# stanFurrer/Robust-Multimodal-Contrastive-Learning

Hardware: AMD Instinct MI355X
Metric: image-text pairs/sec, ViLT-B/32 RMCL step (PGD K=3) (higher is better)
Workload: dtype bf16; 1 GPU; RMCL step, PGD K=3 image attack + MoCo InfoNCE (queue 65536) + full backward + AdamW, ViLT-B/32, bs=64/GPU, 384x384 img + 40 tok (BASELINE configs[2]; [3] when n_gpus=8); global_batch=64, parallelism=dp1, grad_sync=ring/f32, ln_fold=on (shift-robust form)

## Files before the change

include/rmcl.h:

```cpp
#ifndef RMCL_H
#define RMCL_H
#include <stdint.h>
#ifdef __cplusplus
extern "C" {
#endif

#define RMCL_F32 0
#define RMCL_BF16 1

#define RMCL_MODE_INFER 0
#define RMCL_MODE_DATA 1
#define RMCL_MODE_FULL 2
#define RMCL_MODE_CLS_TAIL 16
#define RMCL_MODE_STREAM_ATTN 32

typedef struct rmcl_dims {
  int B;
  int L;
  int P;
  int D;
  int H;
  int layers;
  int mlp;
  int patch_k;
// ... 35 lines not shown
int rmcl_linear_lnfold_c(const void* xb, const void* wf, const float* s, const float* c, const float* part, int nparts, const float* center,
                         void* out, void* preact, int M, int N, int K, int gelu, float eps, float* mean, float* rstd, void* stream);

typedef struct rmcl_chain_stage {
  const void* A; const void* W; const float* bias; const float* residual; void* out; void* out2; float* part; const float* center;
  const float* ln_s; const float* ln_c; float* mean; float* rstd;
  int N, K, epi, nparts; float ln_eps;
} rmcl_chain_stage;
int rmcl_gemm_chain(const rmcl_chain_stage* stages, int n, int M, uint32_t* tickets, uint32_t epoch, int flags, int32_t* xcc, int64_t* stamps,
                    int stamp_wg, void* stream);

int rmcl_l2_prefetch_experiment(const void* A, int64_t lda_bytes, int M, int rows_per_tile, int tiles_per_xcd, int col_tiles, const void* W,
                                int64_t ldw_bytes, int nB, int nk, int tick, int lead, int per_xcd, int wgs, int* counter, int64_t* stamps,
                                void* stream);

typedef struct rmcl_layout {
  int64_t word, pos, btype, eln_w, eln_b;
  int64_t vtype;
  int64_t cls, pos_img, patch_w, patch_b;
  int64_t layer0, layer_stride;
  int64_t ln1_w, ln1_b, qkv_w, qkv_b, proj_w, proj_b, ln2_w, ln2_b, fc1_w, fc1_b, fc2_w, fc2_b;
  int64_t norm_w, norm_b;
  int64_t mh0_w, mh0_b, mh1_w, mh1_b, mh3_w;
  int64_t ema_end;
  int64_t pool_w, pool_b;
  int64_t itm_w, itm_b;
  int64_t total;
} rmcl_layout;

const char* rmcl_last_error(void);
int rmcl_version(void);

int rmcl_tune_set(int key, int value);

int rmcl_grad_ready_wait(int layer, void* stream);
int rmcl_set_side_stream(void* stream);
int rmcl_set_prefetch_stream(void* stream);

int rmcl_dropout_mask_apply(float* x, int64_t n, uint32_t drop_seed, int layer, int site, float drop_p, void* stream);

int rmcl_prof_begin(int tag_mask, int max_launches);
int rmcl_prof_end(double* ms_total, int64_t* launches, double* flops_total);

void rmcl_param_layout(const rmcl_dims* d, rmcl_layout* out);
int64_t rmcl_stash_bytes(const rmcl_dims* d, int mode);
int64_t rmcl_workspace_bytes(const rmcl_dims* d);
int64_t rmcl_heads_stash_bytes(const rmcl_dims* d);


int rmcl_im2patch_f32(const float* img, float* patches, int B, int C, int Hh, int Ww, int ps, int to_image, void* stream);

int rmcl_patch_select(const float* img, int B, int C, int Hh, int Ww, int ps, int32_t* sel, int32_t* counts, int32_t* hw, void* stream);
int rmcl_im2patch_sel(float* img, float* patches, const int32_t* sel, const int32_t* counts, int sel_ld, int B, int n, int C, int Hh,
                      int Ww, int ps, int to_image, void* stream);
int rmcl_image_u8_to_patches(const uint8_t* img, const int32_t* sizes, const int32_t* sel, const int32_t* counts, int sel_ld, int B, int n,
                             int Hmax, int Wmax, int patch_size, const float* lut, float* patches, void* stream);

int rmcl_image_resize_u8(const uint8_t* src, const int32_t* src_sizes, int B, int Hs, int Ws, const int32_t* dst_sizes, int Hd, int Wd,
                         const int32_t* hbounds, const int32_t* hk, int ksh, const int32_t* vbounds, const int32_t* vk, int ksv, uint8_t* tmp,
                         uint8_t* dst, void* stream);

#define RMCL_RA_AUTOCONTRAST 0
#define RMCL_RA_EQUALIZE 1
#define RMCL_RA_ROTATE 2
#define RMCL_RA_POSTERIZE 3
#define RMCL_RA_SOLARIZE 4
// ... 252 lines not shown
```

robust-multimodal-contrastive-learning_amd/_lib.py:

```python
import ctypes as C
import os

import torch

_HERE = os.path.dirname(os.path.abspath(__file__))
LIB_PATH = os.environ.get("RMCL_LIB") or os.path.join(_HERE, "lib", "librmcl_hip.so")

F32, BF16 = 0, 1
MODE_INFER, MODE_DATA, MODE_FULL = 0, 1, 2
MODE_CLS_TAIL = 16
MODE_STREAM_ATTN = 32
PGD_DELTA_ZERO, PGD_SUM_PREV = 1, 2
HEADS_NO_WGRAD = 1
OPTIM_ADAM, OPTIM_SGD = 1, 2
EPI_BIAS, EPI_GELU, EPI_SAVE_PREACT, EPI_RESIDUAL, EPI_DGELU, EPI_ATOMIC, EPI_ACCUM, EPI_TANH = 1, 2, 4, 8, 16, 32, 64, 128
EPI_LNFOLD, EPI_ROWSTAT = 2048, 4096


class Dims(C.Structure):
    _fields_ = [(n, C.c_int) for n in
                ("B", "L", "P", "D", "H", "layers", "mlp", "patch_k", "proj", "vocab", "dtype", "exact", "Pp", "n_types", "img_type")]


class Ragged(C.Structure):
# ... 65 lines not shown


class MetricOps(C.Structure):
    _fields_ = [("n_ops", C.c_int32), ("reserved", C.c_int32), ("op", MetricOp * METRIC_MAX_OPS)]


class RmclError(RuntimeError):
    pass


def _load():
    if not os.path.exists(LIB_PATH):
        raise RmclError(
            f"{LIB_PATH} is missing: build it with `python -c 'import __graft_entry__ as g; g.build()'` "
            "(hipcc --offload-arch=gfx950).  rmcl_amd has no CPU fallback.")
    lib = C.CDLL(LIB_PATH)
    lib.rmcl_last_error.restype = C.c_char_p
    for name in ("rmcl_stash_bytes", "rmcl_workspace_bytes", "rmcl_heads_stash_bytes", "rmcl_infonce_ws_bytes",
                 "rmcl_attention_scratch_elems", "rmcl_attention_stream_stat_elems", "rmcl_ln_fold_elems", "rmcl_bt_stash_floats", "rmcl_bt_loss_ws_floats",
                 "rmcl_vqa_stash_floats", "rmcl_mlm_ws_floats", "rmcl_mpp_ws_floats", "rmcl_randaug_scratch_bytes", "rmcl_grad_stats_ws_bytes"):
        getattr(lib, name).restype = C.c_int64
    lib.rmcl_grad_stats_ws_bytes.argtypes = [C.c_int64]
    lib.rmcl_randaug_scratch_bytes.argtypes = [C.c_int, C.c_int]
    lib.rmcl_randaug_u8.argtypes = [C.c_void_p, C.c_void_p, C.c_int, C.c_int, C.c_int, C.c_void_p, C.c_void_p, C.c_int, C.c_void_p, C.c_void_p, C.c_void_p, C.c_void_p]
    lib.rmcl_mpp_labels_u8.argtypes = [C.c_void_p, C.c_void_p, C.c_int, C.c_int, C.c_int, C.c_void_p, C.c_void_p, C.c_void_p, C.c_int, C.c_int, C.c_int,
                                       C.c_void_p, C.c_void_p]
    lib.rmcl_metrics_update.argtypes = [C.c_void_p, C.c_int, C.POINTER(MetricOps), C.c_void_p]
    return lib


lib = _load()

EXPORTS = (
    "rmcl_last_error", "rmcl_version", "rmcl_prof_begin", "rmcl_prof_end", "rmcl_tune_set", "rmcl_grad_ready_wait", "rmcl_set_side_stream", "rmcl_set_prefetch_stream", "rmcl_dropout_mask_apply", "rmcl_param_layout", "rmcl_ln_fold_elems", "rmcl_ln_fold", "rmcl_linear_rowstat", "rmcl_linear_lnfold", "rmcl_linear_rowstat_c", "rmcl_linear_lnfold_c", "rmcl_weight_transpose_bf16", "rmcl_stash_bytes", "rmcl_workspace_bytes",
    "rmcl_heads_stash_bytes", "rmcl_im2patch_f32", "rmcl_patch_select", "rmcl_im2patch_sel", "rmcl_image_u8_to_patches", "rmcl_image_resize_u8", "rmcl_randaug_scratch_bytes", "rmcl_randaug_u8", "rmcl_add_cast_f32", "rmcl_shard_sum", "rmcl_encoder_forward", "rmcl_encoder_backward",
    "rmcl_heads_forward", "rmcl_heads_forward2", "rmcl_heads_backward", "rmcl_infonce_ws_bytes", "rmcl_infonce_f32", "rmcl_infonce_split_bf16", "rmcl_pgd_step", "rmcl_pgd_step_fused",
    "rmcl_delta_channel_norm", "rmcl_ema_f32", "rmcl_enqueue_f32", "rmcl_cast_f32", "rmcl_adamw_f32", "rmcl_grad_stats_ws_bytes", "rmcl_grad_stats_f32", "rmcl_adamw_guarded_f32", "rmcl_optim_step_f32", "rmcl_ipot_f32", "rmcl_gemm_batched", "rmcl_l2norm_rows_fwd", "rmcl_l2norm_rows_bwd",
    "rmcl_wpa_cost_finish", "rmcl_wpa_distance", "rmcl_itm_fwd", "rmcl_itm_bwd",
    "rmcl_gemm", "rmcl_gemm_rows_bf16", "rmcl_rows_gather_f32", "rmcl_gemm_chain", "rmcl_l2_prefetch_experiment", "rmcl_gemm_route", "rmcl_gemm_kblk", "rmcl_layernorm_fwd", "rmcl_layernorm_bwd", "rmcl_attention_scratch_elems", "rmcl_attention_fwd",
    "rmcl_attention_bwd", "rmcl_attention_stream_stat_elems", "rmcl_attention_stream_fwd", "rmcl_attention_stream_bwd",
    "rmcl_bt_stash_floats", "rmcl_bt_head_forward", "rmcl_bt_head_backward", "rmcl_bt_corr", "rmcl_bt_loss_ws_floats", "rmcl_bt_loss",
    "rmcl_bt_dz", "rmcl_bt_pair_metrics",
    "rmcl_vqa_stash_floats", "rmcl_vqa_head_forward", "rmcl_vqa_bce", "rmcl_vqa_targets_dense", "rmcl_vqa_head_backward",
    "rmcl_nlvr2_ce",
    "rmcl_visual_embed", "rmcl_encoder_forward_rank", "rmcl_irtr_score", "rmcl_irtr_ce", "rmcl_irtr_bwd",
    "rmcl_mlm_ws_floats", "rmcl_mlm_compact", "rmcl_mlm_weight_transpose", "rmcl_mlm_forward", "rmcl_mlm_backward", "rmcl_mlm_logits",
    "rmcl_mpp_ws_floats", "rmcl_mpp_labels", "rmcl_mpp_labels_u8", "rmcl_mpp_compact", "rmcl_mpp_forward", "rmcl_mpp_backward", "rmcl_mpp_logits",
    "rmcl_encoder_forward_mpp", "rmcl_encoder_backward_mpp", "rmcl_visual_embed_mpp",
    "rmcl_word_saliency",
    "rmcl_metrics_update",
)


def check(rc, what=""):
    if rc != 0:
        msg = lib.rmcl_last_error()
        raise RmclError(f"{what} failed (code {rc}): {msg.decode() if msg else '?'}")


def P(t):
    return C.c_void_p(0 if t is None else t.data_ptr())


def I64(v):
    return C.c_int64(int(v))


# ... 3 lines not shown
```

robust-multimodal-contrastive-learning_amd/csrc/api.cpp:

```cpp
#include "rmcl_common.h"
#include "kernels.h"
#include "../../include/rmcl.h"
#include <mutex>
#include <string>
#include <unordered_set>

static thread_local std::string g_err;
extern "C" void rmcl_set_error(const char* msg) { g_err = msg ? msg : ""; }

int rmcl_attention_fwd_impl(const void* qkv, const int* mask, void* out, void* probs, float* scores, int B, int N, int H, int dt,
                            int exact, hipStream_t s);
int rmcl_attention_bwd_impl(const void* qkv, const int* mask, const void* probs, const void* dout, const void* out, void* dqkv,
                            float* scores, void* dS, int B, int N, int H, int dt, int exact, hipStream_t s);

#include <vector>
namespace {
struct Prof {
  bool on = false;
  int mask = 0;
  size_t n = 0, cap = 0;
  std::vector<hipEvent_t> ev;
  double flops = 0.0;
} g_prof;
}
// ... 58 lines not shown
    hipEvent_t e;
    HIP_TRY(hipEventCreate(&e));
    g_prof.ev.push_back(e);
  }
  g_prof.on = true; g_prof.mask = tag_mask; g_prof.n = 0; g_prof.cap = max_launches; g_prof.flops = 0.0;
  return 0;
}
int rmcl_prof_end(double* ms_total, int64_t* launches, double* flops_total) {
  g_prof.on = false;
  double ms = 0.0;
  for (size_t i = 0; i < g_prof.n; ++i) {
    float t = 0.f;
    HIP_TRY(hipEventSynchronize(g_prof.ev[2 * i + 1]));
    HIP_TRY(hipEventElapsedTime(&t, g_prof.ev[2 * i], g_prof.ev[2 * i + 1]));
    ms += t;
  }
  if (ms_total) *ms_total = ms;
  if (launches) *launches = (int64_t)g_prof.n;
  if (flops_total) *flops_total = g_prof.flops;
  return 0;
}
int rmcl_version(void) { return 1; }

int rmcl_dropout_mask_apply(float* x, int64_t n, uint32_t drop_seed, int layer, int site, float drop_p, void* stream) {
  RMCL_REQUIRE(x && drop_p >= 0.f && drop_p < 1.f, "dropout_mask_apply: bad argument");
  if (drop_p == 0.f) return 0;
  return rmcl_dropout_apply(x, n, rmcl_site_seed(drop_seed, layer, site), (uint32_t)((double)drop_p * 4294967296.0), 1.0f / (1.0f - drop_p),
                            (hipStream_t)stream);
}
extern int g_st_reserve_cus;
extern bool g_attn_fused_bwd;
extern bool g_dw_grouped;
extern int g_attn_fwd_waves;
extern int g_infonce_fold;
extern int g_dp_stagger;
extern int g_attn_bwd_persist;
extern int g_attn_bwd_tpw;
extern int g_gemm_share;
extern bool g_lnfold_centred;
extern int g_prefetch_mask, g_prefetch_wgs;
extern int g_st_res_lds;
extern bool g_preact_tiled;
int rmcl_l2_prefetch_experiment(const void* A, int64_t lda_bytes, int M, int rows_per_tile, int tiles_per_xcd, int col_tiles, const void* B,
                                int64_t ldb_bytes, int nB, int nk, int tick, int lead, int per_xcd, int wgs, int* counter, int64_t* stamps, void* stream) {
  RMCL_REQUIRE(A && B && counter && M > 0 && nk > 0 && per_xcd > 0 && wgs > 0 && col_tiles > 0, "l2_prefetch_experiment: bad argument");
  return rmcl_debug_l2_prefetch(A, (long)lda_bytes, M, rows_per_tile, tiles_per_xcd, col_tiles, B, (long)ldb_bytes, nB, nk, tick, lead, per_xcd, wgs, counter,
                                reinterpret_cast<long long*>(stamps), (hipStream_t)stream);
}
int rmcl_tune_set(int key, int value) {
  if (key == 11) { g_lnfold_centred = value != 0; return 0; }
  if (key == 12) { g_prefetch_mask = value & 7; return 0; }
  if (key == 13) { g_prefetch_wgs = value < 0 ? 0 : (value > 64 ? 64 : value); return 0; }
  if (key == 15) { g_preact_tiled = value != 0; return 0; }
  if (key == 14) { g_st_res_lds = value != 0; return 0; }
  if (key == 7) { g_dp_stagger = value < 0 ? 0 : value; return 0; }
  if (key == 10) { g_gemm_share = value < 1 ? 1 : (value > 8 ? 8 : value); return 0; }
  if (key == 9) { g_attn_bwd_tpw = value; return 0; }
  if (key == 8) { g_attn_bwd_persist = value < 0 ? 0 : value; return 0; }
  if (key == 6) { rmcl_gemm_skinny_set_form(value); return 0; }
  if (key == 0) { rmcl_gemm_fast_set_cfg(value); return 0; }
  if (key == 1) { g_st_reserve_cus = value < 0 ? 0 : (value > 128 ? 128 : value); return 0; }
  if (key == 2) { g_attn_fused_bwd = value != 0; return 0; }
  if (key == 5) { g_infonce_fold = value != 0; return 0; }
  if (key == 4) { g_attn_fwd_waves = value; return 0; }
  if (key == 3) { g_dw_grouped = value != 0; return 0; }
  rmcl_set_error("tune_set: unknown key");
  return -1;
}

int64_t rmcl_heads_stash_bytes(const rmcl_dims* d) { return (int64_t)carve_heads(*d, nullptr, nullptr) + 256; }

int rmcl_heads_forward(const rmcl_dims* d, const float* pool32, const float* head32, const float* xn, void* hstash,
                       float* cls_feats, float* q, void* stream) {
  return rmcl_heads_forward2(d, pool32, head32, xn, hstash, cls_feats, q, 0, stream);
}
int rmcl_heads_forward2(const rmcl_dims* d, const float* pool32, const float* head32, const float* xn, void* hstash,
                        float* cls_feats, float* q, int flags, void* stream) {
  RMCL_REQUIRE(d && pool32 && xn && hstash && cls_feats, "heads_forward: NULL argument");
  RMCL_REQUIRE((flags & ~RMCL_HEADS_NO_WGRAD) == 0, "heads_forward: unknown flag");
  rmcl_layout y;
  rmcl_param_layout(d, &y);
  HeadStash h;
  carve_heads(*d, hstash, &h);
  hipStream_t s = (hipStream_t)stream;
  const int B = d->B, D = d->D, N = d->L + 1 + d->P;
  const bool stash_in = !(flags & RMCL_HEADS_NO_WGRAD);
  {
    std::lock_guard<std::mutex> lk(g_nowgrad_mu);
    if (stash_in) g_nowgrad_stash.erase(hstash); else g_nowgrad_stash.insert(hstash);
  }
  if (stash_in) RMCL_TRY(rmcl_gather_rows(xn, h.cls_in, B, D, 1, N, 0, s));
  {
    GemmArgs g = stash_in ? gemm_args(h.cls_in, pool32 + y.pool_w, h.pooled, B, D, D, D, D, D)
                          : gemm_args(xn, pool32 + y.pool_w, h.pooled, B, D, D, N * D, D, D);
    g.epi = EPI_BIAS | EPI_TANH | EPI_DUP; g.bias = pool32 + y.pool_b; g.C2 = cls_feats;
    const bool dup = rmcl_gemm_skinny_supported(g, RMCL_F32, RMCL_F32, 1);
    if (!dup) { g.epi &= ~EPI_DUP; g.C2 = nullptr; }
// ... 371 lines not shown
```

robust-multimodal-contrastive-learning_amd/csrc/attention.hip:

```cpp
#include "rmcl_common.h"
#include "kernels.h"

typedef __bf16 bf16x8 __attribute__((ext_vector_type(8)));
typedef __attribute__((address_space(3))) void lds_void;
typedef const __attribute__((address_space(1))) void glb_void;

#define SCALE 0.125f
#define LOG2E 1.4426950408889634f
#define LN2 0.6931471805599453f
#define SCALE_L2 (SCALE * LOG2E)
int g_attn_fwd_waves = 8;
#define ATT_DQW 8

template <bool TR, int NW = 4>
__device__ __forceinline__ void stage_rows(char* img, const bf16_t* __restrict__ src, long ld, int N, int NKP, int wave, int lane) {
  for (int inst = wave; inst < NKP / 8; inst += NW) {
    const int row = inst * 8 + (lane >> 3), cp = lane & 7;
    int c;
    if (TR) c = (((cp >> 1) ^ ((row >> 1) & 3)) << 1) | (cp & 1);
    else c = cp ^ (row & 7);
    const bf16_t* p = src + (long)min(row, N - 1) * ld + c * 8;
    __builtin_amdgcn_global_load_lds((glb_void*)p, (lds_void*)(img + inst * 1024), 16, 0, 0);
  }
}

__device__ __forceinline__ void touch_line(const void* p, uint32_t sink_lds_addr) {
  uint32_t keep;
  asm volatile("s_mov_b32 %0, m0\n\ts_mov_b32 m0, %2\n\ts_nop 0\n\tglobal_load_lds_dword %1, off\n\ts_mov_b32 m0, %0"
               : "=&s"(keep) : "v"(p), "s"(sink_lds_addr));
}

__device__ __forceinline__ bf16x8 frag_row_lds(const char* img, int row0, int s, int lane) {
  const int row = row0 + (lane & 15);
  const int chunk = (4 * s + (lane >> 4)) ^ (row & 7);
  return *reinterpret_cast<const bf16x8*>(img + row * 128 + chunk * 16);
}

__device__ __forceinline__ bf16x8 frag_row_ldsT(const char* img, int row0, int s, int lane) {
  const int row = row0 + (lane & 15);
  const int c = 4 * s + (lane >> 4);
  const int cp = (((c >> 1) ^ ((row >> 1) & 3)) << 1) | (c & 1);
  return *reinterpret_cast<const bf16x8*>(img + row * 128 + cp * 16);
}

// ... 41 lines not shown
}

__device__ __forceinline__ void fill_maskbias(float* mb, const int* __restrict__ mask, int N, int NKP, int t, int nthreads = 256) {
  for (int j = t; j < NKP; j += nthreads) mb[j] = (j < N && mask[j] != 0) ? 0.f : -INFINITY;
}

#ifdef ST_TRACE
__device__ long long g_at_trace[2][32];
#define AT_STAMP(i)                                                                                              \
  if (blockIdx.x == 300 && (threadIdx.x == 0 || threadIdx.x == 320)) g_at_trace[threadIdx.x != 0][i] = wall_clock64()
extern "C" int rmcl_debug_at_trace(long long* out) {
  return (int)hipMemcpyFromSymbol(out, HIP_SYMBOL(g_at_trace), sizeof(long long) * 64);
}
#define AT_STAMPB(i)                                                                                             \
  if (prob == 300 && (threadIdx.x == 0 || threadIdx.x == 320)) g_at_trace[threadIdx.x != 0][i] = wall_clock64()
#else
#define AT_STAMP(i)
#define AT_STAMPB(i)
#endif

template <int NKT, int ATT_QW>
__global__ __launch_bounds__(ATT_QW * 64) void attn_fwd_kernel(const bf16_t* __restrict__ qkv, const int* __restrict__ mask,
                                                       bf16_t* __restrict__ out, float* __restrict__ lse, int N, int H) {
  extern __shared__ __attribute__((aligned(16))) char sm[];
  constexpr int NKP = NKT * 16;
  char* Kimg = sm;
  char* Vimg = sm + NKP * 128;
  float* mb = reinterpret_cast<float*>(sm + 2 * NKP * 128);
  const int t = threadIdx.x, lane = t & 63, wave = t >> 6, g = lane >> 4;
  const int b = blockIdx.x / H, h = blockIdx.x % H, D = H * 64;
  AT_STAMP(16);
  const long ld = 3 * D;
  const bf16_t* base = qkv + (long)b * N * ld + h * 64;
  bf16x8 qn[2];
  qn[0] = frag_row_global(base, ld, wave * 16, N, 0, lane);
  qn[1] = frag_row_global(base, ld, wave * 16, N, 1, lane);
  stage_rows<false, ATT_QW>(Kimg, base + D, ld, N, NKP, wave, lane);
  stage_rows<true, ATT_QW>(Vimg, base + 2 * D, ld, N, NKP, wave, lane);
  fill_maskbias(mb, mask + (long)b * N, N, NKP, t, ATT_QW * 64);
  AT_STAMP(17);
  const int nqt = (N + 15) / 16;
  AT_STAMP(18);
  __syncthreads();
  AT_STAMP(19);
  for (int qt = wave; qt < nqt; qt += ATT_QW) {
    bf16x8 qf[2] = {qn[0], qn[1]};
    if (qt + ATT_QW < nqt) {
      qn[0] = frag_row_global(base, ld, (qt + ATT_QW) * 16, N, 0, lane);
      qn[1] = frag_row_global(base, ld, (qt + ATT_QW) * 16, N, 1, lane);
    }
    f32x4 S[NKT];
#pragma unroll
    for (int kt = 0; kt < NKT; ++kt) {
      S[kt] = f32x4{0.f, 0.f, 0.f, 0.f};
#pragma unroll
      for (int s = 0; s < 2; ++s) S[kt] = __builtin_amdgcn_mfma_f32_16x16x32_bf16(frag_row_lds(Kimg, kt * 16, s, lane), qf[s], S[kt], 0, 0, 0);
      if (kt & 1) __builtin_amdgcn_sched_barrier(0);
    }
    float m = -INFINITY;
#pragma unroll
    for (int kt = 0; kt < NKT; ++kt) {
      const float4 bias = *reinterpret_cast<const float4*>(mb + kt * 16 + 4 * g);
      S[kt][0] = fmaf(S[kt][0], SCALE_L2, bias.x); S[kt][1] = fmaf(S[kt][1], SCALE_L2, bias.y);
      S[kt][2] = fmaf(S[kt][2], SCALE_L2, bias.z); S[kt][3] = fmaf(S[kt][3], SCALE_L2, bias.w);
      m = fmaxf(m, fmaxf(fmaxf(S[kt][0], S[kt][1]), fmaxf(S[kt][2], S[kt][3])));
    }
    m = group_max(m);
    float l = 0.f;
#pragma unroll
    for (int kt = 0; kt < NKT; ++kt)
#pragma unroll
      for (int r = 0; r < 4; ++r) { S[kt][r] = __builtin_amdgcn_exp2f(S[kt][r] - m); l += S[kt][r]; }
    l = group_sum(l);
    const int q_lane = qt * 16 + (lane & 15);
    if (g == 0 && q_lane < N) lse[((long)blockIdx.x) * NKP + q_lane] = m * LN2 + __logf(l);
    f32x4 O[4];
#pragma unroll
    for (int dt = 0; dt < 4; ++dt) O[dt] = f32x4{0.f, 0.f, 0.f, 0.f};
#pragma unroll
    for (int u = 0; u < NKT / 2; ++u) {
      const bf16x8 pa = pack8(S[2 * u], S[2 * u + 1]);
#pragma unroll
      for (int dt = 0; dt < 4; ++dt) O[dt] = __builtin_amdgcn_mfma_f32_16x16x32_bf16(frag_tr32_lds(Vimg, 32 * u, dt, lane), pa, O[dt], 0, 0, 0);
      __builtin_amdgcn_sched_barrier(0);
    }
    AT_STAMP(20 + (qt >= ATT_QW ? 2 : 0));
    const float linv = 1.0f / l;
    if (q_lane < N) {
      bf16_t* o = out + ((long)b * N + q_lane) * D + h * 64 + 4 * g;
#pragma unroll
      for (int dt = 0; dt < 4; ++dt) {
        uint2 pk;
        pk.x = (uint32_t)f2bf(O[dt][0] * linv) | ((uint32_t)f2bf(O[dt][1] * linv) << 16);
        pk.y = (uint32_t)f2bf(O[dt][2] * linv) | ((uint32_t)f2bf(O[dt][3] * linv) << 16);
        *reinterpret_cast<uint2*>(o + 16 * dt) = pk;
      }
    }
  }
#ifdef ST_TRACE
  AT_STAMP(24);
  asm volatile("s_waitcnt vmcnt(0)" ::: "memory");
  AT_STAMP(25);
#endif
}

template <int NKT>
__global__ __launch_bounds__(ATT_DQW * 64) void attn_bwd_dq_kernel(const bf16_t* __restrict__ qkv, const int* __restrict__ mask,
                                                          const bf16_t* __restrict__ dout, const float* __restrict__ lse,
                                                          float* __restrict__ delta, bf16_t* __restrict__ dqkv, int N, int H) {
  extern __shared__ __attribute__((aligned(16))) char sm[];
  constexpr int NKP = NKT * 16;
  char* Krow = sm;
  char* Vrow = sm + NKP * 128;
  char* Ktr = sm + 2 * NKP * 128;
  float* mb = reinterpret_cast<float*>(sm + 3 * NKP * 128);
  const int t = threadIdx.x, lane = t & 63, wave = t >> 6, g = lane >> 4;
  const int b = blockIdx.x / H, h = blockIdx.x % H, D = H * 64;
  const long ld = 3 * D;
  const bf16_t* base = qkv + (long)b * N * ld + h * 64;
  const bf16_t* dob = dout + (long)b * N * D + h * 64;
  stage_rows<false, ATT_DQW>(Krow, base + D, ld, N, NKP, wave, lane);
  stage_rows<false, ATT_DQW>(Vrow, base + 2 * D, ld, N, NKP, wave, lane);
  stage_rows<true, ATT_DQW>(Ktr, base + D, ld, N, NKP, wave, lane);
  fill_maskbias(mb, mask + (long)b * N, N, NKP, t, ATT_DQW * 64);

  const int nqt = (N + 15) / 16;
  bf16x8 qn[2], dn[2];
  float Ln;
#pragma unroll
// ... 144 lines not shown
#pragma unroll
      for (int r = 0; r < 4; ++r) {
        P[r] = __builtin_amdgcn_exp2f(fmaf(S[r], SCALE_L2, mbk[i] - Lr[r]));
        dS[r] = P[r] * (dP[r] - Dr[r]) * SCALE;
      }
      const s16x4 pa = pack4(P), sa = pack4(dS);
#pragma unroll
      for (int dt = 0; dt < 4; ++dt) {
        dV[i][dt] = __builtin_amdgcn_mfma_f32_16x16x16bf16_1k(dot[dt], pa, dV[i][dt], 0, 0, 0);
        dK[i][dt] = __builtin_amdgcn_mfma_f32_16x16x16bf16_1k(qtr[dt], sa, dK[i][dt], 0, 0, 0);
      }
    }
  }
#pragma unroll
  for (int i = 0; i < TPW; ++i) {
    const int key = (wave + NW * i) * 16 + (lane & 15);
    if (key < N) {
      bf16_t* o = dqkv + ((long)b * N + key) * ld + h * 64 + 4 * g;
#pragma unroll
      for (int dt = 0; dt < 4; ++dt) {
        uint2 pk, pv;
        pk.x = (uint32_t)f2bf(dK[i][dt][0]) | ((uint32_t)f2bf(dK[i][dt][1]) << 16);
        pk.y = (uint32_t)f2bf(dK[i][dt][2]) | ((uint32_t)f2bf(dK[i][dt][3]) << 16);
        pv.x = (uint32_t)f2bf(dV[i][dt][0]) | ((uint32_t)f2bf(dV[i][dt][1]) << 16);
        pv.y = (uint32_t)f2bf(dV[i][dt][2]) | ((uint32_t)f2bf(dV[i][dt][3]) << 16);
        *reinterpret_cast<uint2*>(o + D + 16 * dt) = pk;
        *reinterpret_cast<uint2*>(o + 2 * D + 16 * dt) = pv;
      }
    }
  }
}


template <int NKT, int TPW>
__global__ __launch_bounds__(NKT / TPW * 64) void attn_bwd_fused_kernel(const bf16_t* __restrict__ qkv, const int* __restrict__ mask,
                                                                       const bf16_t* __restrict__ dout, const bf16_t* __restrict__ out,
                                                                       const float* __restrict__ lse, bf16_t* __restrict__ dqkv, int N, int H, int P) {
  extern __shared__ __attribute__((aligned(16))) char sm[];
  constexpr int NKP = NKT * 16, NW = NKT / TPW, NSUB = (NKP + 63) / 64;
  static_assert(NKT % TPW == 0, "key tiles per wave must divide the tile count");
  char* Qtr = sm;
  char* Dtr = sm + NKP * 128;
  char* Ktr = sm + 2 * NKP * 128;
  char* dSimg = sm + 3 * NKP * 128;
  float* Ls = reinterpret_cast<float*>(sm + (3 + NSUB) * NKP * 128);
  float* Ds = Ls + NKP;
  char* touch_sink = reinterpret_cast<char*>(Ds + NKP);
  const int t = threadIdx.x, lane = t & 63, wave = t >> 6, g = lane >> 4;
  const int D = H * 64;
  const long ld = 3 * D;
  for (int prob = blockIdx.x; prob < P; prob += gridDim.x) {
  const int b = prob / H, h = prob % H;
  AT_STAMPB(0);
  const bf16_t* base = qkv + (long)b * N * ld + h * 64;
  const bf16_t* dob = dout + (long)b * N * D + h * 64;
  const bf16_t* ob = out + (long)b * N * D + h * 64;
  bf16x8 kf[TPW][2], vf[TPW][2], of[TPW][2];
  const int* mrow = mask + (long)b * N;
  int mkey[TPW];
#pragma unroll
  for (int i = 0; i < TPW; ++i) mkey[i] = mrow[min((wave * TPW + i) * 16 + (lane & 15), N - 1)];
#pragma unroll
  for (int i = 0; i < TPW; ++i)
#pragma unroll
    for (int s = 0; s < 2; ++s) vf[i][s] = frag_row_global(base + 2 * D, ld, (wave * TPW + i) * 16, N, s, lane);
#pragma unroll
  for (int i = 0; i < TPW; ++i)
// ... 118 lines not shown
    const int off = r * 128 + ((c ^ (r & 7)) * 16);
    const uint2 k0 = *reinterpret_cast<const uint2*>(Qtr + off), k1 = *reinterpret_cast<const uint2*>(Qtr + off + 8);
    const uint2 v0 = *reinterpret_cast<const uint2*>(Dtr + off), v1 = *reinterpret_cast<const uint2*>(Dtr + off + 8);
    if (r < N) {
      bf16_t* o = dqkv + ((long)b * N + r) * ld + h * 64 + c * 8;
      *reinterpret_cast<uint4*>(o + D) = uint4{k0.x, k0.y, k1.x, k1.y};
      *reinterpret_cast<uint4*>(o + 2 * D) = uint4{v0.x, v0.y, v1.x, v1.y};
    }
  }
  AT_STAMPB(7);

  {
    f32x4 dQ[TPW][4];
#pragma unroll
    for (int i = 0; i < TPW; ++i)
#pragma unroll
      for (int dt = 0; dt < 4; ++dt) dQ[i][dt] = f32x4{0.f, 0.f, 0.f, 0.f};
#pragma unroll
    for (int u = 0; u < NKT / 2; ++u) {
      bf16x8 sb[TPW];
#pragma unroll
      for (int i = 0; i < TPW; ++i) {
        const int qt = wave * TPW + i;
        sb[i] = frag_tr32_lds(dSimg + (qt >> 2) * (NKP * 128), 32 * u, qt & 3, lane);
      }
#pragma unroll
      for (int dt = 0; dt < 4; ++dt) {
        const bf16x8 ka = frag_tr32_lds(Ktr, 32 * u, dt, lane);
#pragma unroll
        for (int i = 0; i < TPW; ++i) dQ[i][dt] = __builtin_amdgcn_mfma_f32_16x16x32_bf16(ka, sb[i], dQ[i][dt], 0, 0, 0);
      }
    }
    AT_STAMPB(8);
#pragma unroll
    for (int i = 0; i < TPW; ++i) {
      const int q_lane = (wave * TPW + i) * 16 + (lane & 15);
      if (q_lane < N) {
        bf16_t* o = dqkv + ((long)b * N + q_lane) * ld + h * 64 + 4 * g;
#pragma unroll
        for (int dt = 0; dt < 4; ++dt) {
          uint2 pk;
          pk.x = (uint32_t)f2bf(dQ[i][dt][0]) | ((uint32_t)f2bf(dQ[i][dt][1]) << 16);
          pk.y = (uint32_t)f2bf(dQ[i][dt][2]) | ((uint32_t)f2bf(dQ[i][dt][3]) << 16);
          *reinterpret_cast<uint2*>(o + 16 * dt) = pk;
        }
      }
    }
  }
#ifdef ST_TRACE
  AT_STAMPB(9);
  asm volatile("s_waitcnt vmcnt(0)" ::: "memory");
  AT_STAMPB(10);
#endif
  __syncthreads();
  }
}

static inline int nkt_for(int N) { return N <= 64 ? 4 : N <= 128 ? 8 : N <= 192 ? 12 : 16; }

long rmcl_attn_stat_elems(int B, int H, int N) { return (long)B * H * nkt_for(N) * 16; }

template <int NKT, int QW> static int launch_fwd_w(const bf16_t* qkv, const int* mask, bf16_t* out, float* lse, int B, int N, int H, hipStream_t s) {
  const size_t lds = (size_t)2 * NKT * 16 * 128 + NKT * 16 * 4;
  static RmclLdsOnce once;
  RMCL_TRY(rmcl_set_max_lds(once, reinterpret_cast<const void*>((attn_fwd_kernel<NKT, QW>)), (int)lds));
  RMCL_LAUNCH((attn_fwd_kernel<NKT, QW>), dim3(B * H), dim3(QW * 64), lds, s, qkv, mask, out, lse, N, H);
  RMCL_CHECK_LAUNCH();
  return 0;
}
template <int NKT> static int launch_fwd(const bf16_t* qkv, const int* mask, bf16_t* out, float* lse, int B, int N, int H, hipStream_t s) {
  if (g_attn_fwd_waves == 6) return launch_fwd_w<NKT, 6>(qkv, mask, out, lse, B, N, H, s);
  if (g_attn_fwd_waves == 12) return launch_fwd_w<NKT, 12>(qkv, mask, out, lse, B, N, H, s);
  if (g_attn_fwd_waves == 4) return launch_fwd_w<NKT, 4>(qkv, mask, out, lse, B, N, H, s);
  return launch_fwd_w<NKT, 8>(qkv, mask, out, lse, B, N, H, s);
}
int g_attn_bwd_tpw = 1;
int g_attn_bwd_persist = 0;
bool g_attn_fused_bwd = true;

template <int NKT, int TPW> static int launch_bwd_fused_t(const bf16_t* qkv, const int* mask, const bf16_t* dout, const bf16_t* out, const float* lse,
                                                          bf16_t* dqkv, int B, int N, int H, hipStream_t s) {
  constexpr int NKP = NKT * 16, NSUB = (NKP + 63) / 64, NW = NKT / TPW;
  const size_t lds = (size_t)(3 + NSUB) * NKP * 128 + 2 * NKP * 4 + NW * 256;
  static RmclLdsOnce once;
  RMCL_TRY(rmcl_set_max_lds(once, reinterpret_cast<const void*>(attn_bwd_fused_kernel<NKT, TPW>), (int)lds));
  const int P = B * H, grid = g_attn_bwd_persist > 0 ? min(P, g_attn_bwd_persist) : P;
  RMCL_LAUNCH((attn_bwd_fused_kernel<NKT, TPW>), dim3(grid), dim3(NW * 64), lds, s, qkv, mask, dout, out, lse, dqkv, N, H, P);
  RMCL_CHECK_LAUNCH();
  return 0;
}
template <int NKT> static int launch_bwd_fused(const bf16_t* qkv, const int* mask, const bf16_t* dout, const bf16_t* out, const float* lse,
                                               bf16_t* dqkv, int B, int N, int H, hipStream_t s) {
  if constexpr (NKT % 2 == 0) if (g_attn_bwd_tpw == 2) return launch_bwd_fused_t<NKT, 2>(qkv, mask, dout, out, lse, dqkv, B, N, H, s);
  if constexpr (NKT % 3 == 0) if (g_attn_bwd_tpw == 3) return launch_bwd_fused_t<NKT, 3>(qkv, mask, dout, out, lse, dqkv, B, N, H, s);
  return launch_bwd_fused_t<NKT, 1>(qkv, mask, dout, out, lse, dqkv, B, N, H, s);
}

template <int NKT> static int launch_bwd(const bf16_t* qkv, const int* mask, const bf16_t* dout, const float* lse, float* delta,
                                         bf16_t* dqkv, int B, int N, int H, hipStream_t s) {
  const size_t lds1 = (size_t)3 * NKT * 16 * 128 + NKT * 16 * 4, lds2 = (size_t)2 * NKT * 16 * 128 + 2 * NKT * 16 * 4;
  constexpr int NW = 4;
  static RmclLdsOnce once1, once2;
  RMCL_TRY(rmcl_set_max_lds(once1, reinterpret_cast<const void*>(attn_bwd_dq_kernel<NKT>), (int)lds1));
  RMCL_TRY(rmcl_set_max_lds(once2, reinterpret_cast<const void*>((attn_bwd_dkv_kernel<NKT, NW>)), (int)lds2));
  RMCL_LAUNCH(attn_bwd_dq_kernel<NKT>, dim3(B * H), dim3(ATT_DQW * 64), lds1, s, qkv, mask, dout, lse, delta, dqkv, N, H);
  RMCL_CHECK_LAUNCH();
  RMCL_LAUNCH((attn_bwd_dkv_kernel<NKT, NW>), dim3(B * H), dim3(NW * 64), lds2, s, qkv, mask, dout, lse, delta, dqkv, N, H);
  RMCL_CHECK_LAUNCH();
  return 0;
}

int rmcl_attn_fused_fwd(const void* qkv, const int* mask, void* out, float* lse, int B, int N, int H, hipStream_t s) {
  RMCL_REQUIRE(N >= 1 && N <= 256, "fused attention: N must be <= 256");
  const bf16_t* q = (const bf16_t*)qkv;
  bf16_t* o = (bf16_t*)out;
  switch (nkt_for(N)) {
    case 4: return launch_fwd<4>(q, mask, o, lse, B, N, H, s);
    case 8: return launch_fwd<8>(q, mask, o, lse, B, N, H, s);
    case 12: return launch_fwd<12>(q, mask, o, lse, B, N, H, s);
    default: return launch_fwd<16>(q, mask, o, lse, B, N, H, s);
  }
}
// ... 23 lines not shown
```

Before: 2026 pairs/s.

## Restructure attention fwd softmax/PV pipelining and stage bwd dQ stores via LDS

In the forward attention kernel, the next Q tile prefetch now happens after the QK MFMAs so it shares registers with the current tile. The softmax probabilities are packed to bf16 before the PV loop, and V fragments are double-buffered from LDS so reads overlap the MFMAs. In the fused backward kernel, a new DQ_ROWS path (on by default) writes dQ into swizzled LDS and reads it back so each row is stored to global memory with 16-byte coalesced writes instead of scattered 8-byte ones. This adds an LDS round trip, changes register pressure, and relies on reusing the Qtr buffer without an explicit barrier.

```diff
diff --git a/include/rmcl.h b/include/rmcl.h
--- a/include/rmcl.h
+++ b/include/rmcl.h
@@ -91,6 +91,7 @@
 int rmcl_version(void);
 
 int rmcl_tune_set(int key, int value);
+int rmcl_attention_fwd_waves(int N);
 
 int rmcl_grad_ready_wait(int layer, void* stream);
 int rmcl_set_side_stream(void* stream);
diff --git a/robust-multimodal-contrastive-learning_amd/_lib.py b/robust-multimodal-contrastive-learning_amd/_lib.py
--- a/robust-multimodal-contrastive-learning_amd/_lib.py
+++ b/robust-multimodal-contrastive-learning_amd/_lib.py
@@ -121,7 +121,7 @@
 lib = _load()
 
 EXPORTS = (
-    "rmcl_last_error", "rmcl_version", "rmcl_prof_begin", "rmcl_prof_end", "rmcl_tune_set", "rmcl_grad_ready_wait", "rmcl_set_side_stream", "rmcl_set_prefetch_stream", "rmcl_dropout_mask_apply", "rmcl_param_layout", "rmcl_ln_fold_elems", "rmcl_ln_fold", "rmcl_linear_rowstat", "rmcl_linear_lnfold", "rmcl_linear_rowstat_c", "rmcl_linear_lnfold_c", "rmcl_weight_transpose_bf16", "rmcl_stash_bytes", "rmcl_workspace_bytes",
+    "rmcl_last_error", "rmcl_version", "rmcl_prof_begin", "rmcl_prof_end", "rmcl_tune_set", "rmcl_attention_fwd_waves", "rmcl_grad_ready_wait", "rmcl_set_side_stream", "rmcl_set_prefetch_stream", "rmcl_dropout_mask_apply", "rmcl_param_layout", "rmcl_ln_fold_elems", "rmcl_ln_fold", "rmcl_linear_rowstat", "rmcl_linear_lnfold", "rmcl_linear_rowstat_c", "rmcl_linear_lnfold_c", "rmcl_weight_transpose_bf16", "rmcl_stash_bytes", "rmcl_workspace_bytes",
     "rmcl_heads_stash_bytes", "rmcl_im2patch_f32", "rmcl_patch_select", "rmcl_im2patch_sel", "rmcl_image_u8_to_patches", "rmcl_image_resize_u8", "rmcl_randaug_scratch_bytes", "rmcl_randaug_u8", "rmcl_add_cast_f32", "rmcl_shard_sum", "rmcl_encoder_forward", "rmcl_encoder_backward",
     "rmcl_heads_forward", "rmcl_heads_forward2", "rmcl_heads_backward", "rmcl_infonce_ws_bytes", "rmcl_infonce_f32", "rmcl_infonce_split_bf16", "rmcl_pgd_step", "rmcl_pgd_step_fused",
     "rmcl_delta_channel_norm", "rmcl_ema_f32", "rmcl_enqueue_f32", "rmcl_cast_f32", "rmcl_adamw_f32", "rmcl_grad_stats_ws_bytes", "rmcl_grad_stats_f32", "rmcl_adamw_guarded_f32", "rmcl_optim_step_f32", "rmcl_ipot_f32", "rmcl_gemm_batched", "rmcl_l2norm_rows_fwd", "rmcl_l2norm_rows_bwd",
diff --git a/robust-multimodal-contrastive-learning_amd/csrc/api.cpp b/robust-multimodal-contrastive-learning_amd/csrc/api.cpp
--- a/robust-multimodal-contrastive-learning_amd/csrc/api.cpp
+++ b/robust-multimodal-contrastive-learning_amd/csrc/api.cpp
@@ -114,6 +114,7 @@
 extern bool g_attn_fused_bwd;
 extern bool g_dw_grouped;
 extern int g_attn_fwd_waves;
+extern int g_attn_bwd_dq_rows;
 extern int g_infonce_fold;
 extern int g_dp_stagger;
 extern int g_attn_bwd_persist;
@@ -145,6 +146,7 @@
   if (key == 2) { g_attn_fused_bwd = value != 0; return 0; }
   if (key == 5) { g_infonce_fold = value != 0; return 0; }
   if (key == 4) { g_attn_fwd_waves = value; return 0; }
+  if (key == 16) { g_attn_bwd_dq_rows = value != 0; return 0; }
   if (key == 3) { g_dw_grouped = value != 0; return 0; }
   rmcl_set_error("tune_set: unknown key");
   return -1;
diff --git a/robust-multimodal-contrastive-learning_amd/csrc/attention.hip b/robust-multimodal-contrastive-learning_amd/csrc/attention.hip
--- a/robust-multimodal-contrastive-learning_amd/csrc/attention.hip
+++ b/robust-multimodal-contrastive-learning_amd/csrc/attention.hip
@@ -9,7 +9,7 @@
 #define LOG2E 1.4426950408889634f
 #define LN2 0.6931471805599453f
 #define SCALE_L2 (SCALE * LOG2E)
-int g_attn_fwd_waves = 8;
+int g_attn_fwd_waves = 0;
 #define ATT_DQW 8
 
 template <bool TR, int NW = 4>
@@ -117,9 +117,9 @@
   AT_STAMP(16);
   const long ld = 3 * D;
   const bf16_t* base = qkv + (long)b * N * ld + h * 64;
-  bf16x8 qn[2];
-  qn[0] = frag_row_global(base, ld, wave * 16, N, 0, lane);
-  qn[1] = frag_row_global(base, ld, wave * 16, N, 1, lane);
+  bf16x8 qf[2];
+  qf[0] = frag_row_global(base, ld, wave * 16, N, 0, lane);
+  qf[1] = frag_row_global(base, ld, wave * 16, N, 1, lane);
   stage_rows<false, ATT_QW>(Kimg, base + D, ld, N, NKP, wave, lane);
   stage_rows<true, ATT_QW>(Vimg, base + 2 * D, ld, N, NKP, wave, lane);
   fill_maskbias(mb, mask + (long)b * N, N, NKP, t, ATT_QW * 64);
@@ -129,11 +129,6 @@
   __syncthreads();
   AT_STAMP(19);
   for (int qt = wave; qt < nqt; qt += ATT_QW) {
-    bf16x8 qf[2] = {qn[0], qn[1]};
-    if (qt + ATT_QW < nqt) {
-      qn[0] = frag_row_global(base, ld, (qt + ATT_QW) * 16, N, 0, lane);
-      qn[1] = frag_row_global(base, ld, (qt + ATT_QW) * 16, N, 1, lane);
-    }
     f32x4 S[NKT];
 #pragma unroll
     for (int kt = 0; kt < NKT; ++kt) {
@@ -142,31 +137,48 @@
       for (int s = 0; s < 2; ++s) S[kt] = __builtin_amdgcn_mfma_f32_16x16x32_bf16(frag_row_lds(Kimg, kt * 16, s, lane), qf[s], S[kt], 0, 0, 0);
       if (kt & 1) __builtin_amdgcn_sched_barrier(0);
     }
+    if (qt + ATT_QW < nqt) {
+      qf[0] = frag_row_global(base, ld, (qt + ATT_QW) * 16, N, 0, lane);
+      qf[1] = frag_row_global(base, ld, (qt + ATT_QW) * 16, N, 1, lane);
+    }
     float m = -INFINITY;
 #pragma unroll
     for (int kt = 0; kt < NKT; ++kt) {
-      const float4 bias = *reinterpret_cast<const float4*>(mb + kt * 16 + 4 * g);
-      S[kt][0] = fmaf(S[kt][0], SCALE_L2, bias.x); S[kt][1] = fmaf(S[kt][1], SCALE_L2, bias.y);
-      S[kt][2] = fmaf(S[kt][2], SCALE_L2, bias.z); S[kt][3] = fmaf(S[kt][3], SCALE_L2, bias.w);
+      const f32x4 bias = f4v(*reinterpret_cast<const float4*>(mb + kt * 16 + 4 * g));
+      S[kt] = __builtin_elementwise_fma(S[kt], f32x4{SCALE_L2, SCALE_L2, SCALE_L2, SCALE_L2}, bias);
       m = fmaxf(m, fmaxf(fmaxf(S[kt][0], S[kt][1]), fmaxf(S[kt][2], S[kt][3])));
     }
     m = group_max(m);
     float l = 0.f;
-#pragma unroll
-    for (int kt = 0; kt < NKT; ++kt)
-#pragma unroll
-      for (int r = 0; r < 4; ++r) { S[kt][r] = __builtin_amdgcn_exp2f(S[kt][r] - m); l += S[kt][r]; }
+    bf16x8 pa[NKT / 2];
+    const f32x4 nm = {-m, -m, -m, -m};
+#pragma unroll
+    for (int u = 0; u < NKT / 2; ++u) {
+      f32x4 e0 = S[2 * u] + nm, e1 = S[2 * u + 1] + nm;
+#pragma unroll
+      for (int r = 0; r < 4; ++r) { e0[r] = __builtin_amdgcn_exp2f(e0[r]); l += e0[r]; }
+#pragma unroll
+      for (int r = 0; r < 4; ++r) { e1[r] = __builtin_amdgcn_exp2f(e1[r]); l += e1[r]; }
+      pa[u] = pack8(e0, e1);
+      asm volatile("" : "+v"(pa[u]));
+    }
     l = group_sum(l);
     const int q_lane = qt * 16 + (lane & 15);
     if (g == 0 && q_lane < N) lse[((long)blockIdx.x) * NKP + q_lane] = m * LN2 + __logf(l);
     f32x4 O[4];
+    bf16x8 vf[2][4];
+#pragma unroll
+    for (int dt = 0; dt < 4; ++dt) vf[0][dt] = frag_tr32_lds(Vimg, 0, dt, lane);
 #pragma unroll
     for (int dt = 0; dt < 4; ++dt) O[dt] = f32x4{0.f, 0.f, 0.f, 0.f};
 #pragma unroll
     for (int u = 0; u < NKT / 2; ++u) {
-      const bf16x8 pa = pack8(S[2 * u], S[2 * u + 1]);
-#pragma unroll
-      for (int dt = 0; dt < 4; ++dt) O[dt] = __builtin_amdgcn_mfma_f32_16x16x32_bf16(frag_tr32_lds(Vimg, 32 * u, dt, lane), pa, O[dt], 0, 0, 0);
+      if (u + 1 < NKT / 2) {
+#pragma unroll
+        for (int dt = 0; dt < 4; ++dt) vf[(u + 1) & 1][dt] = frag_tr32_lds(Vimg, 32 * (u + 1), dt, lane);
+      }
+#pragma unroll
+      for (int dt = 0; dt < 4; ++dt) O[dt] = __builtin_amdgcn_mfma_f32_16x16x32_bf16(vf[u & 1][dt], pa[u], O[dt], 0, 0, 0);
       __builtin_amdgcn_sched_barrier(0);
     }
     AT_STAMP(20 + (qt >= ATT_QW ? 2 : 0));
@@ -174,12 +186,7 @@
     if (q_lane < N) {
       bf16_t* o = out + ((long)b * N + q_lane) * D + h * 64 + 4 * g;
 #pragma unroll
-      for (int dt = 0; dt < 4; ++dt) {
-        uint2 pk;
-        pk.x = (uint32_t)f2bf(O[dt][0] * linv) | ((uint32_t)f2bf(O[dt][1] * linv) << 16);
-        pk.y = (uint32_t)f2bf(O[dt][2] * linv) | ((uint32_t)f2bf(O[dt][3] * linv) << 16);
-        *reinterpret_cast<uint2*>(o + 16 * dt) = pk;
-      }
+      for (int dt = 0; dt < 4; ++dt) *reinterpret_cast<uint2*>(o + 16 * dt) = f2bf4(O[dt] * linv);
     }
   }
 #ifdef ST_TRACE
@@ -390,7 +397,7 @@
 }
 
 
-template <int NKT, int TPW>
+template <int NKT, int TPW, bool DQ_ROWS>
 __global__ __launch_bounds__(NKT / TPW * 64) void attn_bwd_fused_kernel(const bf16_t* __restrict__ qkv, const int* __restrict__ mask,
                                                                        const bf16_t* __restrict__ dout, const bf16_t* __restrict__ out,
                                                                        const float* __restrict__ lse, bf16_t* __restrict__ dqkv, int N, int H, int P) {
@@ -575,17 +582,33 @@
       }
     }
     AT_STAMPB(8);
-#pragma unroll
-    for (int i = 0; i < TPW; ++i) {
-      const int q_lane = (wave * TPW + i) * 16 + (lane & 15);
-      if (q_lane < N) {
-        bf16_t* o = dqkv + ((long)b * N + q_lane) * ld + h * 64 + 4 * g;
-#pragma unroll
-        for (int dt = 0; dt < 4; ++dt) {
-          uint2 pk;
-          pk.x = (uint32_t)f2bf(dQ[i][dt][0]) | ((uint32_t)f2bf(dQ[i][dt][1]) << 16);
-          pk.y = (uint32_t)f2bf(dQ[i][dt][2]) | ((uint32_t)f2bf(dQ[i][dt][3]) << 16);
-          *reinterpret_cast<uint2*>(o + 16 * dt) = pk;
+    if constexpr (DQ_ROWS) {
+      int ln = lane;
+      asm volatile("" : "+v"(ln));
+      const int gq = ln >> 4;
+#pragma unroll
+      for (int i = 0; i < TPW; ++i) {
+        const int row = (wave * TPW + i) * 16 + (ln & 15);
+#pragma unroll
+        for (int dt = 0; dt < 4; ++dt)
+          *reinterpret_cast<uint2*>(Qtr + row * 128 + (((2 * dt + (gq >> 1)) ^ (row & 7)) * 16) + (gq & 1) * 8) = f2bf4(dQ[i][dt]);
+      }
+      asm volatile("" ::: "memory");
+#pragma unroll
+      for (int it = 0; it < 2 * TPW; ++it) {
+        const int r = wave * TPW * 16 + it * 8 + (ln >> 3), c = ln & 7;
+        const int off = r * 128 + ((c ^ (r & 7)) * 16);
+        const uint2 q0 = *reinterpret_cast<const uint2*>(Qtr + off), q1 = *reinterpret_cast<const uint2*>(Qtr + off + 8);
+        if (r < N) *reinterpret_cast<uint4*>(dqkv + ((long)b * N + r) * ld + h * 64 + c * 8) = uint4{q0.x, q0.y, q1.x, q1.y};
+      }
+    } else {
+#pragma unroll
+      for (int i = 0; i < TPW; ++i) {
+        const int q_lane = (wave * TPW + i) * 16 + (lane & 15);
+        if (q_lane < N) {
+          bf16_t* o = dqkv + ((long)b * N + q_lane) * ld + h * 64 + 4 * g;
+#pragma unroll
+          for (int dt = 0; dt < 4; ++dt) *reinterpret_cast<uint2*>(o + 16 * dt) = f2bf4(dQ[i][dt]);
         }
       }
     }
@@ -602,6 +625,9 @@
 static inline int nkt_for(int N) { return N <= 64 ? 4 : N <= 128 ? 8 : N <= 192 ? 12 : 16; }
 
 long rmcl_attn_stat_elems(int B, int H, int N) { return (long)B * H * nkt_for(N) * 16; }
+
+static inline int fwd_waves_for(int nkt) { return g_attn_fwd_waves ? g_attn_fwd_waves : 8; }
+extern "C" int rmcl_attention_fwd_waves(int N) { return fwd_waves_for(nkt_for(N)); }
 
 template <int NKT, int QW> static int launch_fwd_w(const bf16_t* qkv, const int* mask, bf16_t* out, float* lse, int B, int N, int H, hipStream_t s) {
   const size_t lds = (size_t)2 * NKT * 16 * 128 + NKT * 16 * 4;
@@ -612,25 +638,32 @@
   return 0;
 }
 template <int NKT> static int launch_fwd(const bf16_t* qkv, const int* mask, bf16_t* out, float* lse, int B, int N, int H, hipStream_t s) {
-  if (g_attn_fwd_waves == 6) return launch_fwd_w<NKT, 6>(qkv, mask, out, lse, B, N, H, s);
-  if (g_attn_fwd_waves == 12) return launch_fwd_w<NKT, 12>(qkv, mask, out, lse, B, N, H, s);
-  if (g_attn_fwd_waves == 4) return launch_fwd_w<NKT, 4>(qkv, mask, out, lse, B, N, H, s);
+  const int waves = fwd_waves_for(NKT);
+  if (waves == 6) return launch_fwd_w<NKT, 6>(qkv, mask, out, lse, B, N, H, s);
+  if (waves == 12) return launch_fwd_w<NKT, 12>(qkv, mask, out, lse, B, N, H, s);
+  if (waves == 4) return launch_fwd_w<NKT, 4>(qkv, mask, out, lse, B, N, H, s);
   return launch_fwd_w<NKT, 8>(qkv, mask, out, lse, B, N, H, s);
 }
 int g_attn_bwd_tpw = 1;
 int g_attn_bwd_persist = 0;
 bool g_attn_fused_bwd = true;
-
-template <int NKT, int TPW> static int launch_bwd_fused_t(const bf16_t* qkv, const int* mask, const bf16_t* dout, const bf16_t* out, const float* lse,
+int g_attn_bwd_dq_rows = 1;
+
+template <int NKT, int TPW, bool DQ_ROWS> static int launch_bwd_fused_d(const bf16_t* qkv, const int* mask, const bf16_t* dout, const bf16_t* out, const float* lse,
                                                           bf16_t* dqkv, int B, int N, int H, hipStream_t s) {
   constexpr int NKP = NKT * 16, NSUB = (NKP + 63) / 64, NW = NKT / TPW;
   const size_t lds = (size_t)(3 + NSUB) * NKP * 128 + 2 * NKP * 4 + NW * 256;
   static RmclLdsOnce once;
-  RMCL_TRY(rmcl_set_max_lds(once, reinterpret_cast<const void*>(attn_bwd_fused_kernel<NKT, TPW>), (int)lds));
+  RMCL_TRY(rmcl_set_max_lds(once, reinterpret_cast<const void*>(attn_bwd_fused_kernel<NKT, TPW, DQ_ROWS>), (int)lds));
   const int P = B * H, grid = g_attn_bwd_persist > 0 ? min(P, g_attn_bwd_persist) : P;
-  RMCL_LAUNCH((attn_bwd_fused_kernel<NKT, TPW>), dim3(grid), dim3(NW * 64), lds, s, qkv, mask, dout, out, lse, dqkv, N, H, P);
+  RMCL_LAUNCH((attn_bwd_fused_kernel<NKT, TPW, DQ_ROWS>), dim3(grid), dim3(NW * 64), lds, s, qkv, mask, dout, out, lse, dqkv, N, H, P);
   RMCL_CHECK_LAUNCH();
   return 0;
+}
+template <int NKT, int TPW> static int launch_bwd_fused_t(const bf16_t* qkv, const int* mask, const bf16_t* dout, const bf16_t* out, const float* lse,
+                                                          bf16_t* dqkv, int B, int N, int H, hipStream_t s) {
+  if (g_attn_bwd_dq_rows) return launch_bwd_fused_d<NKT, TPW, true>(qkv, mask, dout, out, lse, dqkv, B, N, H, s);
+  return launch_bwd_fused_d<NKT, TPW, false>(qkv, mask, dout, out, lse, dqkv, B, N, H, s);
 }
 template <int NKT> static int launch_bwd_fused(const bf16_t* qkv, const int* mask, const bf16_t* dout, const bf16_t* out, const float* lse,
                                                bf16_t* dqkv, int B, int N, int H, hipStream_t s) {
```

Result: no change. 2034 pairs/s (median of 6 runs) (+0.4%).
